# ericehanley/gke-ray-train

Measured on AMD Instinct MI355X. Metric: tokens/sec (whole node) Llama-2-7B fine-tune at 1/2/4/8 MI355X; samples/sec on Wikitext-2, higher is better.
Workload: dtype bf16; 1 GPU; model=llama2-7b, global_batch=8, seq_len=1024, parallelism=dp1, micro_batch=8, grad_accum=1, optimizer=fused AdamW fp32 states, activation_checkpointing=False, optimizer_overlap=True, forced_collectives=False, library_gemms=offline-tuned

## Files before the change

### gke_ray_train_amd/csrc/bindings/ops.cpp

```cpp
#include <climits>
#include <torch/extension.h>

#include <algorithm>
#include <cmath>
#include <c10/hip/HIPStream.h>
#include <c10/core/DeviceGuard.h>

#include "grt_kernels.h"
#include "grt_sdma.h"

namespace {

using at::Tensor;
using c10::optional;

hipStream_t cur_stream(const Tensor& t) {
  return c10::hip::getCurrentHIPStream(t.device().index()).stream();
}

grt::DType dtype_of(const Tensor& t) {
  if (t.scalar_type() == at::kBFloat16) return grt::DType::BF16;
  TORCH_CHECK(t.scalar_type() == at::kFloat, "gke_ray_train_amd kernels support bf16/fp32, got ", t.scalar_type());
  return grt::DType::F32;
}
// ... 21 lines not shown
  check_vec(t, d, name);
  const int64_t vec = t.scalar_type() == at::kBFloat16 ? 8 : 4;
  TORCH_CHECK(d / vec <= grt::norm_max_chunks(), name, ": last dim ", d, " is wider than the norm kernels' limit of ",
              grt::norm_max_chunks(), " 16-byte chunks (", grt::norm_max_chunks() * vec, " elements of ",
              t.scalar_type(), ")");
  return d;
}
void check_norm_like(const Tensor& t, const Tensor& rows_t, const char* name) {
  check_contig(t, name);
  TORCH_CHECK(t.sizes() == rows_t.sizes() && t.scalar_type() == rows_t.scalar_type() && t.device() == rows_t.device(),
              name, " must match the input's shape, dtype and device");
}
void check_norm_param(const Tensor& t, const Tensor& rows_t, int64_t d, const char* name) {
  check_contig(t, name);
  TORCH_CHECK(t.numel() == d && t.scalar_type() == rows_t.scalar_type() && t.device() == rows_t.device(), name,
              " must hold ", d, " elements in the input's dtype on its device");
}
void check_norm_stat(const Tensor& t, const Tensor& rows_t, int64_t rows, const char* name) {
  check_contig(t, name);
  TORCH_CHECK(t.numel() == rows && t.scalar_type() == at::kFloat && t.device() == rows_t.device(), name,
              " must hold one fp32 value per row (", rows, ") on the input's device");
}

std::vector<Tensor> rmsnorm_fwd(const Tensor& x, const optional<Tensor>& residual, const Tensor& w,
                                double eps, int64_t pad) {
  const int64_t d = check_norm_rows(x, "x"), rows = x.numel() / d;
  check_norm_param(w, x, d, "w");
  c10::OptionalDeviceGuard g(x.device());
  TORCH_CHECK(pad >= 0 && pad % 8 == 0 && (pad == 0 || x.dim() == 2), "rmsnorm_fwd: pad % 8 == 0 on [rows, d]");
  auto y = pad == 0 ? at::empty_like(x) : at::empty({rows, d + pad}, x.options()).narrow(1, 0, d);
  auto rstd = at::empty({rows}, x.options().dtype(at::kFloat));
  Tensor h;
  if (residual.has_value()) {
    check_norm_like(*residual, x, "residual");
    h = at::empty_like(x);
  }
  if (rows == 0) return {y, residual.has_value() ? h : x, rstd};
  grt::rmsnorm_fwd(dtype_of(x), x.data_ptr(), ptr_or_null(residual), w.data_ptr(), y.data_ptr(),
                   residual.has_value() ? h.data_ptr() : nullptr, rstd.data_ptr<float>(), rows, (int)d,
                   (float)eps, cur_stream(x), d + pad);
  return {y, residual.has_value() ? h : x, rstd};
}

std::vector<Tensor> rmsnorm_bwd(const Tensor& dy, const Tensor& h, const Tensor& w, const Tensor& rstd,
                                const optional<Tensor>& dres, const optional<Tensor>& dw_out, bool accumulate) {
  const int64_t d = check_norm_rows(h, "h"), rows = h.numel() / d;
  check_norm_like(dy, h, "dy");
  check_norm_param(w, h, d, "w");
  check_norm_stat(rstd, h, rows, "rstd");
  if (dres.has_value()) check_norm_like(*dres, h, "dres");
  if (dw_out.has_value()) check_norm_param(*dw_out, h, d, "dw_out");
  c10::OptionalDeviceGuard g(h.device());
  auto dx = at::empty_like(h);
  if (rows == 0) {
    if (!dw_out.has_value()) return {dx, at::zeros({d}, h.options().dtype(at::kFloat))};
    if (!accumulate) dw_out->zero_();
    return {dx, *dw_out};
  }
  Tensor dw = dw_out.has_value() ? *dw_out : at::empty({d}, h.options().dtype(at::kFloat));
  auto ws = at::empty({grt::norm_bwd_workspace_floats(rows, (int)d)}, h.options().dtype(at::kFloat));
  grt::rmsnorm_bwd(dtype_of(h), dy.data_ptr(), h.data_ptr(), w.data_ptr(), rstd.data_ptr<float>(),
                   ptr_or_null(dres), dx.data_ptr(), dw_out.has_value() ? nullptr : dw.data_ptr<float>(),
                   ws.data_ptr<float>(), rows, (int)d, cur_stream(h),
                   dw_out.has_value() ? dw.data_ptr() : nullptr, accumulate ? 1 : 0);
  return {dx, dw};
}

Tensor rmsnorm_bwd_dx(const Tensor& dy, const Tensor& h, const Tensor& w, const Tensor& rstd,
                      const optional<Tensor>& dres) {
  const int64_t d = check_norm_rows(h, "h"), rows = h.numel() / d;
  check_norm_like(dy, h, "dy");
  check_norm_param(w, h, d, "w");
  check_norm_stat(rstd, h, rows, "rstd");
  if (dres.has_value()) check_norm_like(*dres, h, "dres");
  c10::OptionalDeviceGuard g(h.device());
  auto dx = at::empty_like(h);
  if (rows == 0) return dx;
  grt::rmsnorm_bwd(dtype_of(h), dy.data_ptr(), h.data_ptr(), w.data_ptr(), rstd.data_ptr<float>(),
                   ptr_or_null(dres), dx.data_ptr(), nullptr, nullptr, rows, (int)d, cur_stream(h), nullptr, 0);
  return dx;
}

std::vector<Tensor> layernorm_fwd(const Tensor& x, const optional<Tensor>& residual, const Tensor& w,
                                  const optional<Tensor>& b, double eps) {
  const int64_t d = check_norm_rows(x, "x"), rows = x.numel() / d;
  check_norm_param(w, x, d, "w");
  if (b.has_value()) check_norm_param(*b, x, d, "b");
  c10::OptionalDeviceGuard g(x.device());
  auto y = at::empty_like(x);
  auto mean = at::empty({rows}, x.options().dtype(at::kFloat));
  auto rstd = at::empty({rows}, x.options().dtype(at::kFloat));
  Tensor h;
  if (residual.has_value()) {
    check_norm_like(*residual, x, "residual");
    h = at::empty_like(x);
  }
  if (rows == 0) return {y, residual.has_value() ? h : x, mean, rstd};
  grt::layernorm_fwd(dtype_of(x), x.data_ptr(), ptr_or_null(residual), w.data_ptr(), ptr_or_null(b),
                     y.data_ptr(), residual.has_value() ? h.data_ptr() : nullptr, mean.data_ptr<float>(),
                     rstd.data_ptr<float>(), rows, (int)d, (float)eps, cur_stream(x));
  return {y, residual.has_value() ? h : x, mean, rstd};
}

std::vector<Tensor> layernorm_bwd(const Tensor& dy, const Tensor& h, const Tensor& w, const Tensor& mean,
                                  const Tensor& rstd, const optional<Tensor>& dres) {
  const int64_t d = check_norm_rows(h, "h"), rows = h.numel() / d;
  check_norm_like(dy, h, "dy");
  check_norm_param(w, h, d, "w");
  check_norm_stat(mean, h, rows, "mean");
  check_norm_stat(rstd, h, rows, "rstd");
  if (dres.has_value()) check_norm_like(*dres, h, "dres");
  c10::OptionalDeviceGuard g(h.device());
  auto dx = at::empty_like(h);
  if (rows == 0) {
    auto z = at::zeros({d}, h.options().dtype(at::kFloat));
    return {dx, z, at::zeros_like(z)};
  }
  auto dw = at::empty({d}, h.options().dtype(at::kFloat));
  auto db = at::empty({d}, h.options().dtype(at::kFloat));
  auto ws = at::empty({grt::norm_bwd_workspace_floats(rows, (int)d)}, h.options().dtype(at::kFloat));
  grt::layernorm_bwd(dtype_of(h), dy.data_ptr(), h.data_ptr(), w.data_ptr(), mean.data_ptr<float>(),
                     rstd.data_ptr<float>(), ptr_or_null(dres), dx.data_ptr(), dw.data_ptr<float>(),
                     db.data_ptr<float>(), ws.data_ptr<float>(), rows, (int)d, cur_stream(h));
  return {dx, dw, db};
}

Tensor swiglu_fwd(const Tensor& gu, int64_t pad) {
  check_contig(gu, "gu");
  c10::OptionalDeviceGuard g(gu.device());
  const int64_t two_f = gu.size(-1), rows = gu.numel() / two_f, f = two_f / 2;
  check_vec(gu, f, "gu");
  TORCH_CHECK(pad >= 0 && pad % 8 == 0 && (pad == 0 || gu.dim() == 2), "swiglu_fwd: pad % 8 == 0 on [rows, 2f]");
  auto sizes = gu.sizes().vec();
  sizes.back() = f;
  auto out = pad == 0 ? at::empty(sizes, gu.options()) : at::empty({rows, f + pad}, gu.options()).narrow(1, 0, f);
  grt::swiglu_fwd(dtype_of(gu), gu.data_ptr(), out.data_ptr(), rows, (int)f, cur_stream(gu), f + pad);
  return out;
}
Tensor swiglu_bwd(const Tensor& gu, const Tensor& dout) {
  check_contig(gu, "gu");
  check_contig(dout, "dout");
  c10::OptionalDeviceGuard g(gu.device());
  const int64_t two_f = gu.size(-1), rows = gu.numel() / two_f, f = two_f / 2;
// ... 1630 lines not shown
    any = any || words[i] != 0;
  }
  TORCH_CHECK(any, "cu_masked_stream: mask selects no CU");
  c10::DeviceGuard g(c10::Device(c10::DeviceType::CUDA, (c10::DeviceIndex)device));
  hipStream_t s = nullptr;
  const hipError_t e = hipExtStreamCreateWithCUMask(&s, (uint32_t)words.size(), words.data());
  TORCH_CHECK(e == hipSuccess, "hipExtStreamCreateWithCUMask: ", hipGetErrorString(e));
  return reinterpret_cast<int64_t>(s);
}

std::vector<int64_t> stream_cu_mask(int64_t stream, int64_t words) {
  TORCH_CHECK(words > 0 && words <= 64, "stream_cu_mask: 1..64 words");
  std::vector<uint32_t> w((size_t)words, 0u);
  const hipError_t e = hipExtStreamGetCUMask(reinterpret_cast<hipStream_t>(stream), (uint32_t)words, w.data());
  TORCH_CHECK(e == hipSuccess, "hipExtStreamGetCUMask: ", hipGetErrorString(e));
  return std::vector<int64_t>(w.begin(), w.end());
}

}

PYBIND11_MODULE(TORCH_EXTENSION_NAME, m) {
  m.doc() = "gke_ray_train_amd HIP kernels for gfx950 (MI355X)";
  m.def("rmsnorm_fwd", &rmsnorm_fwd, py::arg("x"), py::arg("residual"), py::arg("w"), py::arg("eps"),
        py::arg("pad") = 0);
  m.def("rmsnorm_bwd", &rmsnorm_bwd, py::arg("dy"), py::arg("h"), py::arg("w"), py::arg("rstd"), py::arg("dres"),
        py::arg("dw_out") = py::none(), py::arg("accumulate") = false);
  m.def("layernorm_fwd", &layernorm_fwd);
  m.def("layernorm_bwd", &layernorm_bwd);
  m.def("swiglu_fwd", &swiglu_fwd, py::arg("gu"), py::arg("pad") = 0);
  m.def("swiglu_bwd", &swiglu_bwd);
  m.def("gelu_fwd", &gelu_fwd);
  m.def("gelu_bwd", &gelu_bwd);
  m.def("rope_fwd", &rope_fwd);
  m.def("rope_bwd", &rope_bwd);
  m.def("rope_append", &rope_append);
  m.def("rope_append_fp8", &rope_append_fp8, py::arg("qkv"), py::arg("cos"), py::arg("sin"), py::arg("pos"), py::arg("hq"),
        py::arg("hkv"), py::arg("D"), py::arg("S"), py::arg("kc"), py::arg("vc"), py::arg("k_scale"), py::arg("v_scale"),
        py::arg("tpr"), py::arg("k_out") = py::none());
  m.def("kv_fp8_dequant", &kv_fp8_dequant);
  m.def("scale_add_pe", &scale_add_pe);
  m.def("dropout_fwd", &dropout_fwd);
  m.def("dropout_bwd", &dropout_bwd);
  m.def("dropout_fwd_seeded", &dropout_fwd_seeded);
  m.def("lora_down", &lora_down, py::arg("x"), py::arg("a"), py::arg("p"), py::arg("seed"), py::arg("offset"),
        py::arg("want_xd"), py::arg("h_out") = py::none(), py::arg("hscale") = 1.0);
  m.def("lora_dx", &lora_dx, py::arg("g"), py::arg("at"), py::arg("dx"), py::arg("p"), py::arg("seed"),
        py::arg("offset"), py::arg("accumulate"), py::arg("dx_in") = py::none(), py::arg("gscale") = 1.0);
  m.def("lora_refresh", &lora_refresh, py::arg("bs"), py::arg("offs"), py::arg("w"), py::arg("wt"), py::arg("col0"),
        py::arg("wt_row0") = -1);
  m.def("lora_g", &lora_g, py::arg("a"), py::arg("bt"), py::arg("c"), py::arg("alpha"), py::arg("accumulate"));
  m.def("lora_g_group", &lora_g_group, py::arg("a"), py::arg("bt"), py::arg("c"), py::arg("alpha"),
// ... 32 lines not shown
        py::arg("rope_sin") = py::none(), py::arg("cu_seqlens") = py::none(), py::arg("max_seqlen") = 0,
        py::arg("dqkv_t") = py::none());
  m.def("rope_attn_fwd_d64", &rope_attn_fwd_d64, py::arg("qkv"), py::arg("cos"), py::arg("sin"), py::arg("o"),
        py::arg("B"), py::arg("S"), py::arg("hq"), py::arg("hkv"), py::arg("scale"), py::arg("causal"),
        py::arg("cu_seqlens") = py::none(), py::arg("max_seqlen") = 0,
        "bf16 head_dim 64: RoPE + flash attention straight from the fused QKV rows (packed with cu_seqlens) -> lse");
  m.def("rope_attn_bwd_d64", &rope_attn_bwd_d64, py::arg("do"), py::arg("qkv"), py::arg("cos"), py::arg("sin"),
        py::arg("o"), py::arg("lse"), py::arg("dqkv"), py::arg("B"), py::arg("S"), py::arg("hq"), py::arg("hkv"),
        py::arg("scale"), py::arg("causal"), py::arg("cu_seqlens") = py::none(), py::arg("max_seqlen") = 0,
        "backward of rope_attn_fwd_d64: un-rotated dQ / dK and dV into the columns of dqkv (every element written)");
  m.def("attn_set_schedule", &grt::attn_set_schedule,
        "bf16 attention causal-pair / XCD-grouped schedule, bit mask: 1 = forward, 2 = dQ, 4 = dK/dV");
  m.def("attn_get_schedule", &grt::attn_get_schedule);
  m.def("attn_set_dkdv_form", &grt::attn_set_dkdv_form, "dK / dV kernel: 1 = 4-wave, 2 = wave-pair (default)");
  m.def("attn_get_dkdv_form", &grt::attn_get_dkdv_form);
  m.def("attn_set_dma_fast", &grt::attn_set_dma_fast, "1 = hoisted LDS-DMA addressing (default), 0 = clamped per tile");
  m.def("ew_set_fast", &grt::ew_set_fast, "1 = single-pass RoPE (D = 128) / SwiGLU kernels (default), 0 = grid-stride kernels");
  m.def("attn_set_skip_dead", &grt::attn_set_skip_dead,
        "1 = forward / dK-dV waves skip the causal tiles they mask entirely (default), 0 = compute them");
  m.def("nf4_quantize", &nf4_quantize);
  m.def("nf4_dequantize", &nf4_dequantize);
  m.def("nf4_dequantize_t", &nf4_dequantize_t);
  m.def("nf4_dequantize_into", &nf4_dequantize_into);
  m.def("rmsnorm_bwd_dx", &rmsnorm_bwd_dx);
  m.def("swiglu_fwd_t", &swiglu_fwd_t);
  m.def("swiglu_bwd_t", &swiglu_bwd_t);
  m.def("transpose_into", &transpose_into);
  m.def("copy_sdma", &copy_sdma);
  m.def("sdma_d2h", &sdma_d2h, py::arg("dst"), py::arg("src"), py::arg("producer_stream") = 0,
        "pinned host <- device on an SDMA engine, ordered on the source's current stream; producer_stream "
        "(a raw stream handle): the stream whose work so far wrote src");
  m.def("sdma_stats", &sdma_stats, "copies / bytes / worker busy seconds / first error of the SDMA copier");
  m.def("sdma_clear_error", [](int64_t device) { grt::sdma_clear_error((int)device); });
  m.def("gemv", &gemv, py::arg("x"), py::arg("w"), py::arg("swiglu") = false);
  m.def("gemv_fused", &gemv_fused, py::arg("x"), py::arg("w"), py::arg("sumsq"), py::arg("slot"),
        py::arg("swiglu") = false, py::arg("g") = py::none(), py::arg("res") = py::none(), py::arg("eps") = 1e-5,
        py::arg("cos") = py::none(), py::arg("sin") = py::none(), py::arg("pos") = py::none(),
        py::arg("kc") = py::none(), py::arg("vc") = py::none(), py::arg("hq") = 0, py::arg("hkv") = 0);
  m.def("nf4_gemv", &nf4_gemv, py::arg("x"), py::arg("qweight"), py::arg("absmax"), py::arg("N"), py::arg("K"),
        py::arg("h") = py::none(), py::arg("lora_b") = py::none(), py::arg("lora_off") = py::none(),
        py::arg("scaling") = 1.0);
  m.def("sample_logits", &sample_logits, py::arg("logits"), py::arg("do_sample") = false, py::arg("temperature") = 1.0,
        py::arg("top_k") = 0, py::arg("top_p") = 1.0, py::arg("seed") = 0, py::arg("counter") = py::none(),
        py::arg("keep_mask") = py::none(), py::arg("finished") = py::none(), py::arg("finish_step") = py::none(),
        py::arg("step") = py::none(), py::arg("next_ids") = py::none(), py::arg("out") = py::none(),
        py::arg("eos_ids") = py::none(), py::arg("pad_id") = py::none(), py::arg("max_steps") = 1,
        py::arg("candidates") = false);
// ... 34 lines not shown
```

### gke_ray_train_amd/csrc/include/grt_kernels.h

```cpp
#pragma once
#include <hip/hip_runtime.h>
#include <stdint.h>

namespace grt {

enum class DType : int { F32 = 0, BF16 = 1 };

void rmsnorm_fwd(DType dt, const void* x, const void* residual, const void* w, void* y, void* h_out,
                 float* rstd, int64_t rows, int d, float eps, hipStream_t s,
                 int64_t ldy = 0);
void rmsnorm_bwd(DType dt, const void* dy, const void* h, const void* w, const float* rstd,
                 const void* dres, void* dx, float* dw_f32, float* ws, int64_t rows, int d,
                 hipStream_t s, void* dw_t = nullptr, int accumulate = 0);
int64_t norm_bwd_workspace_floats(int64_t rows, int d);
int norm_max_chunks();
void layernorm_fwd(DType dt, const void* x, const void* residual, const void* w, const void* b,
                   void* y, void* h_out, float* mean, float* rstd, int64_t rows, int d, float eps,
                   hipStream_t s);
void layernorm_bwd(DType dt, const void* dy, const void* h, const void* w, const float* mean,
                   const float* rstd, const void* dres, void* dx, float* dw_f32, float* db_f32,
                   float* ws, int64_t rows, int d, hipStream_t s);

void swiglu_fwd(DType dt, const void* gu, void* out, int64_t rows, int f, hipStream_t s, int64_t ldo = 0);
bool swiglu_fwd_t(const void* gu, void* out, void* outT, int64_t rows, int f, hipStream_t s, int64_t ldo = 0);
bool swiglu_bwd_t(const void* gu, const void* dout, void* dgu, void* dguT, int64_t rows, int f, hipStream_t s);
void swiglu_bwd(DType dt, const void* gu, const void* dout, void* dgu, int64_t rows, int f,
                hipStream_t s);
void gelu_fwd(DType dt, const void* x, void* y, int64_t n, hipStream_t s);
void gelu_bwd(DType dt, const void* x, const void* dy, void* dx, int64_t n, hipStream_t s);
void ew_set_fast(int on);
void rope_fwd(DType dt, const void* qkv, int64_t ld, void* q_out, void* k_out, const float* cos,
              const float* sin, const int32_t* pos, int64_t T, int S, int hq, int hkv, int D,
              hipStream_t s);
void rope_append(const void* qkv, int64_t ld, void* q_out, void* kc, void* vc, int64_t c_bs, int64_t c_ss,
                 int64_t c_hs, int64_t v_bs, int64_t v_ss, int64_t v_hs, const float* cos, const float* sin,
                 const int32_t* pos, int64_t T_, int tpr, int S, int L, int hq, int hkv, int D, hipStream_t s);
void rope_bwd(DType dt, const void* dq, const void* dk, void* dqkv, int64_t ld, const float* cos,
// ... 344 lines not shown
```

### gke_ray_train_amd/csrc/kernels/norm.hip

```cpp
#include <stdlib.h>

#include "grt_common.h"
#include "grt_kernels.h"

namespace grt {
namespace {

constexpr int kNT = 256;
constexpr int kRowsPerBlock = kNT / kWave;
constexpr int kBwdMaxBlocks = 512;

template <typename T, int MAXC, bool RMS, bool RES, bool FULL>
__global__ __launch_bounds__(kNT) void norm_fwd_kernel(const T* __restrict__ x,
                                                       const T* __restrict__ res,
                                                       const T* __restrict__ w,
                                                       const T* __restrict__ b, T* __restrict__ y,
                                                       T* __restrict__ h_out, float* __restrict__ mean_out,
                                                       float* __restrict__ rstd_out, int64_t rows,
                                                       int d, float eps, int64_t ldy) {
  constexpr int V = Vec16<T>::N;
  typedef typename Vec16<T>::type VT;
  const int lane = threadIdx.x & 63;
  const int64_t row = (int64_t)blockIdx.x * kRowsPerBlock + (threadIdx.x >> 6);
  if (row >= rows) return;
  const int nchunk = d / V;
  const T* xr = x + row * d;
  const T* rr = RES ? res + row * d : nullptr;
  VT xv[MAXC], rv[MAXC], wvv[MAXC];
#pragma unroll
  for (int c = 0; c < MAXC; ++c) {
    const int ch = FULL ? lane + c * kWave : min(lane + c * kWave, nchunk - 1);
    xv[c] = *reinterpret_cast<const VT*>(xr + ch * V);
    if (RES) rv[c] = *reinterpret_cast<const VT*>(rr + ch * V);
  }
#pragma unroll
  for (int c = 0; c < MAXC; ++c) {
    const int ch = FULL ? lane + c * kWave : min(lane + c * kWave, nchunk - 1);
    wvv[c] = *reinterpret_cast<const VT*>(w + ch * V);
  }
  float hv[MAXC][V];
  float s1 = 0.f;
#pragma unroll
  for (int c = 0; c < MAXC; ++c) {
    const bool ok = FULL || lane + c * kWave < nchunk;
#pragma unroll
    for (int i = 0; i < V; ++i) {
      float t = to_f(xv[c][i]);
      if (RES) t = to_f(from_f<T>(t + to_f(rv[c][i])));
      hv[c][i] = ok ? t : 0.f;
      s1 += RMS ? hv[c][i] * hv[c][i] : hv[c][i];
    }
    if (RES && ok) store16(h_out + row * d + (lane + c * kWave) * V, hv[c]);
  }
  s1 = wave_sum(s1);
  float mu = 0.f, rstd;
  if (RMS) {
    rstd = rsqrtf(s1 / d + eps);
  } else {
    mu = s1 / d;
    float s2 = 0.f;
#pragma unroll
    for (int c = 0; c < MAXC; ++c) {
      const bool ok = FULL || lane + c * kWave < nchunk;
#pragma unroll
      for (int i = 0; i < V; ++i) { const float t = hv[c][i] - mu; s2 += ok ? t * t : 0.f; }
    }
    s2 = wave_sum(s2);
    rstd = rsqrtf(s2 / d + eps);
  }
#pragma unroll
  for (int c = 0; c < MAXC; ++c) {
    const int ch = lane + c * kWave;
    if (FULL || ch < nchunk) {
      float o[V];
      if (!RMS && b != nullptr) {
        float bv[V];
        load16(b + ch * V, bv);
#pragma unroll
        for (int i = 0; i < V; ++i) o[i] = (hv[c][i] - mu) * rstd * to_f(wvv[c][i]) + bv[i];
      } else {
#pragma unroll
        for (int i = 0; i < V; ++i) o[i] = (hv[c][i] - mu) * rstd * to_f(wvv[c][i]);
      }
      store16(y + row * ldy + ch * V, o);
    }
  }
  if (lane == 0) {
    rstd_out[row] = rstd;
    if (!RMS) mean_out[row] = mu;
  }
}

template <typename T, int MAXC, bool RMS, bool RES>
__global__ __launch_bounds__(kNT) void norm_bwd_kernel(const T* __restrict__ dy,
                                                       const T* __restrict__ h,
                                                       const T* __restrict__ w,
                                                       const float* __restrict__ mean,
                                                       const float* __restrict__ rstd,
                                                       const T* __restrict__ dres, T* __restrict__ dx,
                                                       float* __restrict__ ws, int64_t rows, int d) {
  constexpr int V = Vec16<T>::N;
  typedef typename Vec16<T>::type VT;
  __shared__ float red[2 * kRowsPerBlock];
  const int tid = threadIdx.x, lane = tid & 63, wid = tid >> 6;
  const int nchunk = d / V;
  float dwp[MAXC][V], dbp[MAXC][V], wv[MAXC][V];
  int chs[MAXC];
#pragma unroll
  for (int c = 0; c < MAXC; ++c) {
    chs[c] = min(tid + c * kNT, nchunk - 1);
#pragma unroll
    for (int i = 0; i < V; ++i) { dwp[c][i] = 0.f; dbp[c][i] = 0.f; }
    load16(w + chs[c] * V, wv[c]);
  }
  VT hn[MAXC], dn[MAXC], rn[MAXC];
  auto load_row = [&](int64_t rr) {
    rr = rr < rows ? rr : rows - 1;
#pragma unroll
    for (int c = 0; c < MAXC; ++c) {
      hn[c] = *reinterpret_cast<const VT*>(h + rr * d + chs[c] * V);
      dn[c] = *reinterpret_cast<const VT*>(dy + rr * d + chs[c] * V);
      if (RES) rn[c] = *reinterpret_cast<const VT*>(dres + rr * d + chs[c] * V);
    }
  };
  load_row(blockIdx.x);
  for (int64_t row = blockIdx.x; row < rows; row += gridDim.x) {
    VT hc[MAXC], dc[MAXC], rc[MAXC];
#pragma unroll
    for (int c = 0; c < MAXC; ++c) { hc[c] = hn[c]; dc[c] = dn[c]; if (RES) rc[c] = rn[c]; }
    load_row(row + gridDim.x);
    const float r = rstd[row];
    const float mu = RMS ? 0.f : mean[row];
    float xh[MAXC][V], g[MAXC][V];
    float sg = 0.f, sgx = 0.f;
#pragma unroll
    for (int c = 0; c < MAXC; ++c) {
      const bool ok = tid + c * kNT < nchunk;
#pragma unroll
      for (int i = 0; i < V; ++i) {
        const float dv = ok ? to_f(dc[c][i]) : 0.f;
        xh[c][i] = (to_f(hc[c][i]) - mu) * r;
        g[c][i] = dv * wv[c][i];
        sg += g[c][i];
        sgx += g[c][i] * xh[c][i];
        dwp[c][i] += dv * xh[c][i];
        if (!RMS) dbp[c][i] += dv;
      }
    }
    sgx = wave_sum(sgx);
    if (!RMS) sg = wave_sum(sg);
    if (lane == 0) { red[wid] = sgx; red[kRowsPerBlock + wid] = sg; }
    __syncthreads();
    float tsgx = 0.f, tsg = 0.f;
#pragma unroll
    for (int i = 0; i < kRowsPerBlock; ++i) { tsgx += red[i]; tsg += red[kRowsPerBlock + i]; }
    __syncthreads();
    tsgx /= d;
    tsg = RMS ? 0.f : tsg / d;
#pragma unroll
    for (int c = 0; c < MAXC; ++c) {
      const int ch = tid + c * kNT;
      if (ch < nchunk) {
        float o[V];
#pragma unroll
        for (int i = 0; i < V; ++i) o[i] = (RES ? to_f(rc[c][i]) : 0.f) + r * (g[c][i] - tsg - xh[c][i] * tsgx);
        store16(dx + row * d + ch * V, o);
      }
    }
  }
  if (ws == nullptr) return;
  float* wsb = ws + (int64_t)blockIdx.x * 2 * d;
#pragma unroll
  for (int c = 0; c < MAXC; ++c) {
    const int ch = tid + c * kNT;
    if (ch < nchunk) {
#pragma unroll
      for (int i = 0; i < V; ++i) {
        wsb[ch * V + i] = dwp[c][i];
        wsb[d + ch * V + i] = dbp[c][i];
      }
    }
  }
}

constexpr int kColsumCols = 16;
constexpr int kColsumGroups = kNT / kColsumCols;
template <typename GO, bool ACC>
__global__ __launch_bounds__(kNT) void colsum_kernel(const float* __restrict__ ws, int nb, int d, int ncols,
                                                     GO* __restrict__ dw, GO* __restrict__ db) {
  __shared__ float red[kColsumGroups][kColsumCols];
  const int c = threadIdx.x % kColsumCols, rg = threadIdx.x / kColsumCols;
  const int j = blockIdx.x * kColsumCols + c;
  float a0 = 0.f, a1 = 0.f, a2 = 0.f, a3 = 0.f;
  if (j < ncols) {
    const int64_t ld = 2 * (int64_t)d;
    constexpr int G = kColsumGroups;
    int b = rg;
    for (; b + 3 * G < nb; b += 4 * G) {
      a0 += ws[(int64_t)b * ld + j];
      a1 += ws[(int64_t)(b + G) * ld + j];
      a2 += ws[(int64_t)(b + 2 * G) * ld + j];
      a3 += ws[(int64_t)(b + 3 * G) * ld + j];
    }
    for (; b < nb; b += G) a0 += ws[(int64_t)b * ld + j];
  }
  red[rg][c] = (a0 + a1) + (a2 + a3);
  __syncthreads();
  if (rg == 0 && j < ncols) {
    float s = 0.f;
#pragma unroll
    for (int g = 0; g < kColsumGroups; ++g) s += red[g][c];
    GO* out = j < d ? dw : db;
    const int jj = j < d ? j : j - d;
    if (out) out[jj] = from_f<GO>(ACC ? to_f(out[jj]) + s : s);
  }
}

constexpr int kNormMaxFwdPerLane = 32;
constexpr int kNormMaxBwdPerThr = 8;
constexpr int kNormMaxChunks = kNormMaxFwdPerLane * kWave;
static_assert(kNormMaxChunks == kNormMaxBwdPerThr * kNT, "forward and backward ladders cover the same width");

template <typename T, bool RMS>
void launch_fwd(const void* x, const void* res, const void* w, const void* b, void* y, void* h_out,
                float* mean, float* rstd, int64_t rows, int d, float eps, hipStream_t s, int64_t ldy = 0) {
  if (ldy <= 0) ldy = d;
  constexpr int V = Vec16<T>::N;
  const int per_lane = (d / V + kWave - 1) / kWave;
  const dim3 grid((unsigned)((rows + kRowsPerBlock - 1) / kRowsPerBlock));
#define GRT_NF4(MC, RES, FULL)                                                                  \
  hipLaunchKernelGGL((norm_fwd_kernel<T, MC, RMS, RES, FULL>), grid, dim3(kNT), 0, s, (const T*)x, \
                     (const T*)res, (const T*)w, (const T*)b, (T*)y, (T*)h_out, mean, rstd, rows,     \
                     d, eps, ldy)
#define GRT_NF(MC)                                                     \
  do {                                                                 \
    const bool full = (d / V) == (MC) * kWave;                         \
    if (res != nullptr) { if (full) GRT_NF4(MC, true, true); else GRT_NF4(MC, true, false); }   \
    else { if (full) GRT_NF4(MC, false, true); else GRT_NF4(MC, false, false); }              \
  } while (0)
  if (per_lane <= 1) GRT_NF(1);
  else if (per_lane <= 2) GRT_NF(2);
  else if (per_lane <= 4) GRT_NF(4);
  else if (per_lane <= 8) GRT_NF(8);
  else if (per_lane <= 16) GRT_NF(16);
  else GRT_NF(kNormMaxFwdPerLane);
#undef GRT_NF
#undef GRT_NF4
}

int bwd_max_blocks() {
  static const int v = [] {
    const char* e = getenv("GRT_NORM_BWD_BLOCKS");
    const int n = e ? atoi(e) : kBwdMaxBlocks;
    return n > 0 ? n : kBwdMaxBlocks;
  }();
  return v;
}

int bwd_blocks(int64_t rows) {
  const int mb = bwd_max_blocks();
  return (int)(rows < mb ? (rows > 0 ? rows : 1) : mb);
}

template <typename T, bool RMS>
void launch_bwd(const void* dy, const void* h, const void* w, const float* mean, const float* rstd,
                const void* dres, void* dx, float* dw, float* db, float* ws, int64_t rows, int d,
                hipStream_t s, void* dw_t = nullptr, int accumulate = 0) {
  constexpr int V = Vec16<T>::N;
  const int per_thr = (d / V + kNT - 1) / kNT;
  const int nb = bwd_blocks(rows);
  const size_t lds = 0;
#define GRT_NB2(MC, RES)                                                                            \
  hipLaunchKernelGGL((norm_bwd_kernel<T, MC, RMS, RES>), dim3(nb), dim3(kNT), lds, s, (const T*)dy, \
                     (const T*)h, (const T*)w, mean, rstd, (const T*)dres, (T*)dx, ws, rows, d)
#define GRT_NB(MC)                                      \
  do {                                                  \
    if (dres != nullptr) GRT_NB2(MC, true);             \
    else GRT_NB2(MC, false);                            \
  } while (0)
  if (per_thr <= 1) GRT_NB(1);
  else if (per_thr <= 2) GRT_NB(2);
  else if (per_thr <= 4) GRT_NB(4);
  else GRT_NB(kNormMaxBwdPerThr);
#undef GRT_NB
#undef GRT_NB2
  if (ws == nullptr) return;
  const int ncols = RMS ? d : 2 * d;
  const dim3 cg((ncols + kColsumCols - 1) / kColsumCols);
  if (dw_t != nullptr && RMS) {
    if (accumulate)
      hipLaunchKernelGGL((colsum_kernel<T, true>), cg, dim3(kNT), 0, s, ws, nb, d, ncols, (T*)dw_t, (T*)nullptr);
    else
      hipLaunchKernelGGL((colsum_kernel<T, false>), cg, dim3(kNT), 0, s, ws, nb, d, ncols, (T*)dw_t, (T*)nullptr);
  } else {
    hipLaunchKernelGGL((colsum_kernel<float, false>), cg, dim3(kNT), 0, s, ws, nb, d, ncols, dw, db);
  }
}

}

int norm_max_chunks() { return kNormMaxChunks; }

int64_t norm_bwd_workspace_floats(int64_t rows, int d) { return (int64_t)bwd_blocks(rows) * 2 * d; }

void rmsnorm_fwd(DType dt, const void* x, const void* residual, const void* w, void* y, void* h_out,
                 float* rstd, int64_t rows, int d, float eps, hipStream_t s, int64_t ldy) {
  if (dt == DType::BF16)
    launch_fwd<bf16, true>(x, residual, w, nullptr, y, h_out, nullptr, rstd, rows, d, eps, s, ldy);
  else
    launch_fwd<float, true>(x, residual, w, nullptr, y, h_out, nullptr, rstd, rows, d, eps, s, ldy);
}

void rmsnorm_bwd(DType dt, const void* dy, const void* h, const void* w, const float* rstd,
                 const void* dres, void* dx, float* dw_f32, float* ws, int64_t rows, int d,
                 hipStream_t s, void* dw_t, int accumulate) {
  if (dt == DType::BF16)
    launch_bwd<bf16, true>(dy, h, w, nullptr, rstd, dres, dx, dw_f32, nullptr, ws, rows, d, s, dw_t, accumulate);
  else
    launch_bwd<float, true>(dy, h, w, nullptr, rstd, dres, dx, dw_f32, nullptr, ws, rows, d, s, dw_t, accumulate);
}

void layernorm_fwd(DType dt, const void* x, const void* residual, const void* w, const void* b,
                   void* y, void* h_out, float* mean, float* rstd, int64_t rows, int d, float eps,
                   hipStream_t s) {
  if (dt == DType::BF16)
    launch_fwd<bf16, false>(x, residual, w, b, y, h_out, mean, rstd, rows, d, eps, s);
// ... 15 lines not shown
```

Before: 28060 tokens/s.

## Make norm kernels persistent with row prefetch, multi-row bwd, vectorized colsum

The forward norm kernel now runs on a capped persistent grid, prefetching the next row's inputs while the current row reduces. It also keeps the residual sum in bf16 registers instead of fp32. The backward kernel handles two rows per iteration for small widths, compiles out the dw path when no workspace is given, and stores only the dw half of the workspace for RMSNorm. The column-sum kernel switches to 1024 threads with float4 loads and shuffle reductions. Optional output buffers are added to the bindings so callers can reuse allocations; this adds register pressure and more complex code paths in the norm kernels, which are a small share of step time.

```diff
diff --git a/gke_ray_train_amd/csrc/bindings/ops.cpp b/gke_ray_train_amd/csrc/bindings/ops.cpp
--- a/gke_ray_train_amd/csrc/bindings/ops.cpp
+++ b/gke_ray_train_amd/csrc/bindings/ops.cpp
@@ -67,18 +67,27 @@
               " must hold one fp32 value per row (", rows, ") on the input's device");
 }
 
+Tensor norm_out(const optional<Tensor>& out, const Tensor& rows_t, const char* name) {
+  if (!out.has_value()) return at::empty_like(rows_t);
+  check_norm_like(*out, rows_t, name);
+  TORCH_CHECK(reinterpret_cast<uintptr_t>(out->data_ptr()) % 16 == 0, name, " must be 16-byte aligned");
+  return *out;
+}
+
 std::vector<Tensor> rmsnorm_fwd(const Tensor& x, const optional<Tensor>& residual, const Tensor& w,
-                                double eps, int64_t pad) {
+                                double eps, int64_t pad, const optional<Tensor>& y_out,
+                                const optional<Tensor>& h_out) {
   const int64_t d = check_norm_rows(x, "x"), rows = x.numel() / d;
   check_norm_param(w, x, d, "w");
   c10::OptionalDeviceGuard g(x.device());
   TORCH_CHECK(pad >= 0 && pad % 8 == 0 && (pad == 0 || x.dim() == 2), "rmsnorm_fwd: pad % 8 == 0 on [rows, d]");
-  auto y = pad == 0 ? at::empty_like(x) : at::empty({rows, d + pad}, x.options()).narrow(1, 0, d);
+  TORCH_CHECK(pad == 0 || !y_out.has_value(), "rmsnorm_fwd: y_out only with pad == 0");
+  auto y = pad == 0 ? norm_out(y_out, x, "y_out") : at::empty({rows, d + pad}, x.options()).narrow(1, 0, d);
   auto rstd = at::empty({rows}, x.options().dtype(at::kFloat));
   Tensor h;
   if (residual.has_value()) {
     check_norm_like(*residual, x, "residual");
-    h = at::empty_like(x);
+    h = norm_out(h_out, x, "h_out");
   }
   if (rows == 0) return {y, residual.has_value() ? h : x, rstd};
   grt::rmsnorm_fwd(dtype_of(x), x.data_ptr(), ptr_or_null(residual), w.data_ptr(), y.data_ptr(),
@@ -88,7 +97,8 @@
 }
 
 std::vector<Tensor> rmsnorm_bwd(const Tensor& dy, const Tensor& h, const Tensor& w, const Tensor& rstd,
-                                const optional<Tensor>& dres, const optional<Tensor>& dw_out, bool accumulate) {
+                                const optional<Tensor>& dres, const optional<Tensor>& dw_out, bool accumulate,
+                                const optional<Tensor>& dx_out) {
   const int64_t d = check_norm_rows(h, "h"), rows = h.numel() / d;
   check_norm_like(dy, h, "dy");
   check_norm_param(w, h, d, "w");
@@ -96,14 +106,14 @@
   if (dres.has_value()) check_norm_like(*dres, h, "dres");
   if (dw_out.has_value()) check_norm_param(*dw_out, h, d, "dw_out");
   c10::OptionalDeviceGuard g(h.device());
-  auto dx = at::empty_like(h);
+  auto dx = norm_out(dx_out, h, "dx_out");
   if (rows == 0) {
     if (!dw_out.has_value()) return {dx, at::zeros({d}, h.options().dtype(at::kFloat))};
     if (!accumulate) dw_out->zero_();
     return {dx, *dw_out};
   }
   Tensor dw = dw_out.has_value() ? *dw_out : at::empty({d}, h.options().dtype(at::kFloat));
-  auto ws = at::empty({grt::norm_bwd_workspace_floats(rows, (int)d)}, h.options().dtype(at::kFloat));
+  auto ws = at::empty({grt::norm_bwd_workspace_floats(rows, (int)d, true)}, h.options().dtype(at::kFloat));
   grt::rmsnorm_bwd(dtype_of(h), dy.data_ptr(), h.data_ptr(), w.data_ptr(), rstd.data_ptr<float>(),
                    ptr_or_null(dres), dx.data_ptr(), dw_out.has_value() ? nullptr : dw.data_ptr<float>(),
                    ws.data_ptr<float>(), rows, (int)d, cur_stream(h),
@@ -112,33 +122,37 @@
 }
 
 Tensor rmsnorm_bwd_dx(const Tensor& dy, const Tensor& h, const Tensor& w, const Tensor& rstd,
-                      const optional<Tensor>& dres) {
+                      const optional<Tensor>& dres, const optional<Tensor>& dx_out) {
   const int64_t d = check_norm_rows(h, "h"), rows = h.numel() / d;
   check_norm_like(dy, h, "dy");
   check_norm_param(w, h, d, "w");
   check_norm_stat(rstd, h, rows, "rstd");
   if (dres.has_value()) check_norm_like(*dres, h, "dres");
   c10::OptionalDeviceGuard g(h.device());
-  auto dx = at::empty_like(h);
+  auto dx = norm_out(dx_out, h, "dx_out");
   if (rows == 0) return dx;
   grt::rmsnorm_bwd(dtype_of(h), dy.data_ptr(), h.data_ptr(), w.data_ptr(), rstd.data_ptr<float>(),
                    ptr_or_null(dres), dx.data_ptr(), nullptr, nullptr, rows, (int)d, cur_stream(h), nullptr, 0);
   return dx;
 }
 
+int64_t norm_fwd_max_waves() { return grt::norm_fwd_max_waves(); }
+int64_t norm_bwd_blocks(int64_t rows) { return grt::norm_bwd_blocks(rows); }
+
 std::vector<Tensor> layernorm_fwd(const Tensor& x, const optional<Tensor>& residual, const Tensor& w,
-                                  const optional<Tensor>& b, double eps) {
+                                  const optional<Tensor>& b, double eps, const optional<Tensor>& y_out,
+                                  const optional<Tensor>& h_out) {
   const int64_t d = check_norm_rows(x, "x"), rows = x.numel() / d;
   check_norm_param(w, x, d, "w");
   if (b.has_value()) check_norm_param(*b, x, d, "b");
   c10::OptionalDeviceGuard g(x.device());
-  auto y = at::empty_like(x);
+  auto y = norm_out(y_out, x, "y_out");
   auto mean = at::empty({rows}, x.options().dtype(at::kFloat));
   auto rstd = at::empty({rows}, x.options().dtype(at::kFloat));
   Tensor h;
   if (residual.has_value()) {
     check_norm_like(*residual, x, "residual");
-    h = at::empty_like(x);
+    h = norm_out(h_out, x, "h_out");
   }
   if (rows == 0) return {y, residual.has_value() ? h : x, mean, rstd};
   grt::layernorm_fwd(dtype_of(x), x.data_ptr(), ptr_or_null(residual), w.data_ptr(), ptr_or_null(b),
@@ -148,7 +162,7 @@
 }
 
 std::vector<Tensor> layernorm_bwd(const Tensor& dy, const Tensor& h, const Tensor& w, const Tensor& mean,
-                                  const Tensor& rstd, const optional<Tensor>& dres) {
+                                  const Tensor& rstd, const optional<Tensor>& dres, const optional<Tensor>& dx_out) {
   const int64_t d = check_norm_rows(h, "h"), rows = h.numel() / d;
   check_norm_like(dy, h, "dy");
   check_norm_param(w, h, d, "w");
@@ -156,14 +170,14 @@
   check_norm_stat(rstd, h, rows, "rstd");
   if (dres.has_value()) check_norm_like(*dres, h, "dres");
   c10::OptionalDeviceGuard g(h.device());
-  auto dx = at::empty_like(h);
+  auto dx = norm_out(dx_out, h, "dx_out");
   if (rows == 0) {
     auto z = at::zeros({d}, h.options().dtype(at::kFloat));
     return {dx, z, at::zeros_like(z)};
   }
   auto dw = at::empty({d}, h.options().dtype(at::kFloat));
   auto db = at::empty({d}, h.options().dtype(at::kFloat));
-  auto ws = at::empty({grt::norm_bwd_workspace_floats(rows, (int)d)}, h.options().dtype(at::kFloat));
+  auto ws = at::empty({grt::norm_bwd_workspace_floats(rows, (int)d, false)}, h.options().dtype(at::kFloat));
   grt::layernorm_bwd(dtype_of(h), dy.data_ptr(), h.data_ptr(), w.data_ptr(), mean.data_ptr<float>(),
                      rstd.data_ptr<float>(), ptr_or_null(dres), dx.data_ptr(), dw.data_ptr<float>(),
                      db.data_ptr<float>(), ws.data_ptr<float>(), rows, (int)d, cur_stream(h));
@@ -1840,11 +1854,15 @@
 PYBIND11_MODULE(TORCH_EXTENSION_NAME, m) {
   m.doc() = "gke_ray_train_amd HIP kernels for gfx950 (MI355X)";
   m.def("rmsnorm_fwd", &rmsnorm_fwd, py::arg("x"), py::arg("residual"), py::arg("w"), py::arg("eps"),
-        py::arg("pad") = 0);
+        py::arg("pad") = 0, py::arg("y_out") = py::none(), py::arg("h_out") = py::none());
   m.def("rmsnorm_bwd", &rmsnorm_bwd, py::arg("dy"), py::arg("h"), py::arg("w"), py::arg("rstd"), py::arg("dres"),
-        py::arg("dw_out") = py::none(), py::arg("accumulate") = false);
-  m.def("layernorm_fwd", &layernorm_fwd);
-  m.def("layernorm_bwd", &layernorm_bwd);
+        py::arg("dw_out") = py::none(), py::arg("accumulate") = false, py::arg("dx_out") = py::none());
+  m.def("layernorm_fwd", &layernorm_fwd, py::arg("x"), py::arg("residual"), py::arg("w"), py::arg("b"), py::arg("eps"),
+        py::arg("y_out") = py::none(), py::arg("h_out") = py::none());
+  m.def("norm_fwd_max_waves", &norm_fwd_max_waves);
+  m.def("norm_bwd_blocks", &norm_bwd_blocks);
+  m.def("layernorm_bwd", &layernorm_bwd, py::arg("dy"), py::arg("h"), py::arg("w"), py::arg("mean"), py::arg("rstd"),
+        py::arg("dres"), py::arg("dx_out") = py::none());
   m.def("swiglu_fwd", &swiglu_fwd, py::arg("gu"), py::arg("pad") = 0);
   m.def("swiglu_bwd", &swiglu_bwd);
   m.def("gelu_fwd", &gelu_fwd);
@@ -1923,7 +1941,8 @@
   m.def("nf4_dequantize", &nf4_dequantize);
   m.def("nf4_dequantize_t", &nf4_dequantize_t);
   m.def("nf4_dequantize_into", &nf4_dequantize_into);
-  m.def("rmsnorm_bwd_dx", &rmsnorm_bwd_dx);
+  m.def("rmsnorm_bwd_dx", &rmsnorm_bwd_dx, py::arg("dy"), py::arg("h"), py::arg("w"), py::arg("rstd"), py::arg("dres"),
+        py::arg("dx_out") = py::none());
   m.def("swiglu_fwd_t", &swiglu_fwd_t);
   m.def("swiglu_bwd_t", &swiglu_bwd_t);
   m.def("transpose_into", &transpose_into);
diff --git a/gke_ray_train_amd/csrc/include/grt_kernels.h b/gke_ray_train_amd/csrc/include/grt_kernels.h
--- a/gke_ray_train_amd/csrc/include/grt_kernels.h
+++ b/gke_ray_train_amd/csrc/include/grt_kernels.h
@@ -12,7 +12,9 @@
 void rmsnorm_bwd(DType dt, const void* dy, const void* h, const void* w, const float* rstd,
                  const void* dres, void* dx, float* dw_f32, float* ws, int64_t rows, int d,
                  hipStream_t s, void* dw_t = nullptr, int accumulate = 0);
-int64_t norm_bwd_workspace_floats(int64_t rows, int d);
+int64_t norm_bwd_workspace_floats(int64_t rows, int d, bool rms);
+int norm_bwd_blocks(int64_t rows);
+int norm_fwd_max_waves();
 int norm_max_chunks();
 void layernorm_fwd(DType dt, const void* x, const void* residual, const void* w, const void* b,
                    void* y, void* h_out, float* mean, float* rstd, int64_t rows, int d, float eps,
diff --git a/gke_ray_train_amd/csrc/kernels/norm.hip b/gke_ray_train_amd/csrc/kernels/norm.hip
--- a/gke_ray_train_amd/csrc/kernels/norm.hip
+++ b/gke_ray_train_amd/csrc/kernels/norm.hip
@@ -9,6 +9,14 @@
 constexpr int kNT = 256;
 constexpr int kRowsPerBlock = kNT / kWave;
 constexpr int kBwdMaxBlocks = 512;
+constexpr int kFwdMaxBlocks = 512;
+
+template <typename VT>
+__device__ __forceinline__ void use16(VT& v) {
+  u32x4 t = __builtin_bit_cast(u32x4, v);
+  asm volatile("" : "+v"(t));
+  v = __builtin_bit_cast(VT, t);
+}
 
 template <typename T, int MAXC, bool RMS, bool RES, bool FULL>
 __global__ __launch_bounds__(kNT) void norm_fwd_kernel(const T* __restrict__ x,
@@ -20,78 +28,99 @@
                                                        int d, float eps, int64_t ldy) {
   constexpr int V = Vec16<T>::N;
   typedef typename Vec16<T>::type VT;
+  constexpr bool PF = MAXC <= 8;
   const int lane = threadIdx.x & 63;
-  const int64_t row = (int64_t)blockIdx.x * kRowsPerBlock + (threadIdx.x >> 6);
+  const int64_t nwave = (int64_t)gridDim.x * kRowsPerBlock;
+  int64_t row = (int64_t)blockIdx.x * kRowsPerBlock + (threadIdx.x >> 6);
   if (row >= rows) return;
   const int nchunk = d / V;
-  const T* xr = x + row * d;
-  const T* rr = RES ? res + row * d : nullptr;
-  VT xv[MAXC], rv[MAXC], wvv[MAXC];
+  const bool bias = !RMS && b != nullptr;
+  int chs[MAXC];
+  VT xn[MAXC], rn[MAXC], wvv[MAXC], bvv[MAXC];
+#pragma unroll
+  for (int c = 0; c < MAXC; ++c) chs[c] = FULL ? lane + c * kWave : min(lane + c * kWave, nchunk - 1);
+  auto load_row = [&](int64_t r) {
+    r = r < rows ? r : rows - 1;
+#pragma unroll
+    for (int c = 0; c < MAXC; ++c) {
+      xn[c] = *reinterpret_cast<const VT*>(x + r * d + chs[c] * V);
+      if (RES) rn[c] = *reinterpret_cast<const VT*>(res + r * d + chs[c] * V);
+    }
+  };
 #pragma unroll
   for (int c = 0; c < MAXC; ++c) {
-    const int ch = FULL ? lane + c * kWave : min(lane + c * kWave, nchunk - 1);
-    xv[c] = *reinterpret_cast<const VT*>(xr + ch * V);
-    if (RES) rv[c] = *reinterpret_cast<const VT*>(rr + ch * V);
-  }
-#pragma unroll
-  for (int c = 0; c < MAXC; ++c) {
-    const int ch = FULL ? lane + c * kWave : min(lane + c * kWave, nchunk - 1);
-    wvv[c] = *reinterpret_cast<const VT*>(w + ch * V);
-  }
-  float hv[MAXC][V];
-  float s1 = 0.f;
-#pragma unroll
-  for (int c = 0; c < MAXC; ++c) {
-    const bool ok = FULL || lane + c * kWave < nchunk;
-#pragma unroll
-    for (int i = 0; i < V; ++i) {
-      float t = to_f(xv[c][i]);
-      if (RES) t = to_f(from_f<T>(t + to_f(rv[c][i])));
-      hv[c][i] = ok ? t : 0.f;
-      s1 += RMS ? hv[c][i] * hv[c][i] : hv[c][i];
-    }
-    if (RES && ok) store16(h_out + row * d + (lane + c * kWave) * V, hv[c]);
-  }
-  s1 = wave_sum(s1);
-  float mu = 0.f, rstd;
-  if (RMS) {
-    rstd = rsqrtf(s1 / d + eps);
-  } else {
-    mu = s1 / d;
-    float s2 = 0.f;
+    wvv[c] = *reinterpret_cast<const VT*>(w + chs[c] * V);
+    if (!RMS) bvv[c] = *reinterpret_cast<const VT*>((bias ? b : w) + chs[c] * V);
+  }
+  if (PF) {
+    load_row(row);
+#pragma unroll
+    for (int c = 0; c < MAXC; ++c) {
+      use16(xn[c]);
+      if (RES) use16(rn[c]);
+    }
+  }
+  for (; row < rows; row += nwave) {
+    if (!PF) load_row(row);
+    VT hb[MAXC];
+    float s1 = 0.f;
 #pragma unroll
     for (int c = 0; c < MAXC; ++c) {
       const bool ok = FULL || lane + c * kWave < nchunk;
 #pragma unroll
-      for (int i = 0; i < V; ++i) { const float t = hv[c][i] - mu; s2 += ok ? t * t : 0.f; }
-    }
-    s2 = wave_sum(s2);
-    rstd = rsqrtf(s2 / d + eps);
-  }
-#pragma unroll
-  for (int c = 0; c < MAXC; ++c) {
-    const int ch = lane + c * kWave;
-    if (FULL || ch < nchunk) {
-      float o[V];
-      if (!RMS && b != nullptr) {
-        float bv[V];
-        load16(b + ch * V, bv);
-#pragma unroll
-        for (int i = 0; i < V; ++i) o[i] = (hv[c][i] - mu) * rstd * to_f(wvv[c][i]) + bv[i];
-      } else {
-#pragma unroll
-        for (int i = 0; i < V; ++i) o[i] = (hv[c][i] - mu) * rstd * to_f(wvv[c][i]);
-      }
-      store16(y + row * ldy + ch * V, o);
-    }
-  }
-  if (lane == 0) {
-    rstd_out[row] = rstd;
-    if (!RMS) mean_out[row] = mu;
-  }
-}
-
-template <typename T, int MAXC, bool RMS, bool RES>
+      for (int i = 0; i < V; ++i) {
+        float t = to_f(xn[c][i]);
+        if (RES) t = to_f(from_f<T>(t + to_f(rn[c][i])));
+        t = ok ? t : 0.f;
+        hb[c][i] = from_f<T>(t);
+        s1 += RMS ? t * t : t;
+      }
+      if (RES && ok) *reinterpret_cast<VT*>(h_out + row * d + (lane + c * kWave) * V) = hb[c];
+    }
+    if (PF) {
+      __builtin_amdgcn_sched_barrier(0);
+      load_row(row + nwave);
+      __builtin_amdgcn_sched_barrier(0);
+    }
+    s1 = wave_sum(s1);
+    float mu = 0.f, rstd;
+    if (RMS) {
+      rstd = rsqrtf(s1 / d + eps);
+    } else {
+      mu = s1 / d;
+      float s2 = 0.f;
+#pragma unroll
+      for (int c = 0; c < MAXC; ++c) {
+        const bool ok = FULL || lane + c * kWave < nchunk;
+#pragma unroll
+        for (int i = 0; i < V; ++i) { const float t = to_f(hb[c][i]) - mu; s2 += ok ? t * t : 0.f; }
+      }
+      s2 = wave_sum(s2);
+      rstd = rsqrtf(s2 / d + eps);
+    }
+#pragma unroll
+    for (int c = 0; c < MAXC; ++c) {
+      const int ch = lane + c * kWave;
+      if (FULL || ch < nchunk) {
+        float o[V];
+        if (bias) {
+#pragma unroll
+          for (int i = 0; i < V; ++i) o[i] = (to_f(hb[c][i]) - mu) * rstd * to_f(wvv[c][i]) + to_f(bvv[c][i]);
+        } else {
+#pragma unroll
+          for (int i = 0; i < V; ++i) o[i] = (to_f(hb[c][i]) - mu) * rstd * to_f(wvv[c][i]);
+        }
+        store16(y + row * ldy + ch * V, o);
+      }
+    }
+    if (lane == 0) {
+      rstd_out[row] = rstd;
+      if (!RMS) mean_out[row] = mu;
+    }
+  }
+}
+
+template <typename T, int MAXC, bool RMS, bool RES, bool DW>
 __global__ __launch_bounds__(kNT) void norm_bwd_kernel(const T* __restrict__ dy,
                                                        const T* __restrict__ h,
                                                        const T* __restrict__ w,
@@ -100,10 +129,12 @@
                                                        const T* __restrict__ dres, T* __restrict__ dx,
                                                        float* __restrict__ ws, int64_t rows, int d) {
   constexpr int V = Vec16<T>::N;
+  constexpr int NR = MAXC <= 2 ? 2 : 1;
   typedef typename Vec16<T>::type VT;
-  __shared__ float red[2 * kRowsPerBlock];
+  __shared__ float red[2 * NR * kRowsPerBlock];
   const int tid = threadIdx.x, lane = tid & 63, wid = tid >> 6;
   const int nchunk = d / V;
+  const int64_t G = gridDim.x;
   float dwp[MAXC][V], dbp[MAXC][V], wv[MAXC][V];
   int chs[MAXC];
 #pragma unroll
@@ -113,63 +144,100 @@
     for (int i = 0; i < V; ++i) { dwp[c][i] = 0.f; dbp[c][i] = 0.f; }
     load16(w + chs[c] * V, wv[c]);
   }
-  VT hn[MAXC], dn[MAXC], rn[MAXC];
-  auto load_row = [&](int64_t rr) {
-    rr = rr < rows ? rr : rows - 1;
-#pragma unroll
-    for (int c = 0; c < MAXC; ++c) {
-      hn[c] = *reinterpret_cast<const VT*>(h + rr * d + chs[c] * V);
-      dn[c] = *reinterpret_cast<const VT*>(dy + rr * d + chs[c] * V);
-      if (RES) rn[c] = *reinterpret_cast<const VT*>(dres + rr * d + chs[c] * V);
+  VT hn[NR][MAXC], dn[NR][MAXC], rn[NR][MAXC];
+  auto load_rows = [&](int64_t r0) {
+#pragma unroll
+    for (int k = 0; k < NR; ++k) {
+      int64_t rr = r0 + k * G;
+      rr = rr < rows ? rr : rows - 1;
+#pragma unroll
+      for (int c = 0; c < MAXC; ++c) {
+        hn[k][c] = *reinterpret_cast<const VT*>(h + rr * d + chs[c] * V);
+        dn[k][c] = *reinterpret_cast<const VT*>(dy + rr * d + chs[c] * V);
+        if (RES) rn[k][c] = *reinterpret_cast<const VT*>(dres + rr * d + chs[c] * V);
+      }
     }
   };
-  load_row(blockIdx.x);
-  for (int64_t row = blockIdx.x; row < rows; row += gridDim.x) {
-    VT hc[MAXC], dc[MAXC], rc[MAXC];
-#pragma unroll
-    for (int c = 0; c < MAXC; ++c) { hc[c] = hn[c]; dc[c] = dn[c]; if (RES) rc[c] = rn[c]; }
-    load_row(row + gridDim.x);
-    const float r = rstd[row];
-    const float mu = RMS ? 0.f : mean[row];
-    float xh[MAXC][V], g[MAXC][V];
-    float sg = 0.f, sgx = 0.f;
-#pragma unroll
-    for (int c = 0; c < MAXC; ++c) {
-      const bool ok = tid + c * kNT < nchunk;
-#pragma unroll
-      for (int i = 0; i < V; ++i) {
-        const float dv = ok ? to_f(dc[c][i]) : 0.f;
-        xh[c][i] = (to_f(hc[c][i]) - mu) * r;
-        g[c][i] = dv * wv[c][i];
-        sg += g[c][i];
-        sgx += g[c][i] * xh[c][i];
-        dwp[c][i] += dv * xh[c][i];
-        if (!RMS) dbp[c][i] += dv;
-      }
-    }
-    sgx = wave_sum(sgx);
-    if (!RMS) sg = wave_sum(sg);
-    if (lane == 0) { red[wid] = sgx; red[kRowsPerBlock + wid] = sg; }
+  load_rows(blockIdx.x);
+  for (int64_t row = blockIdx.x; row < rows; row += NR * G) {
+    VT hc[NR][MAXC], dc[NR][MAXC], rc[NR][MAXC];
+#pragma unroll
+    for (int k = 0; k < NR; ++k) {
+#pragma unroll
+      for (int c = 0; c < MAXC; ++c) { hc[k][c] = hn[k][c]; dc[k][c] = dn[k][c]; if (RES) rc[k][c] = rn[k][c]; }
+    }
+    load_rows(row + NR * G);
+    float r[NR], mu[NR], sg[NR], sgx[NR];
+    float xh[NR][MAXC][V], g[NR][MAXC][V];
+#pragma unroll
+    for (int k = 0; k < NR; ++k) {
+      const bool live = row + k * G < rows;
+      const int64_t rk = live ? row + k * G : row;
+      r[k] = rstd[rk];
+      mu[k] = RMS ? 0.f : mean[rk];
+      sg[k] = 0.f;
+      sgx[k] = 0.f;
+#pragma unroll
+      for (int c = 0; c < MAXC; ++c) {
+        const bool ok = tid + c * kNT < nchunk;
+#pragma unroll
+        for (int i = 0; i < V; ++i) {
+          const float dv = ok ? to_f(dc[k][c][i]) : 0.f;
+          xh[k][c][i] = (to_f(hc[k][c][i]) - mu[k]) * r[k];
+          g[k][c][i] = dv * wv[c][i];
+          sg[k] += g[k][c][i];
+          sgx[k] += g[k][c][i] * xh[k][c][i];
+          if (DW) {
+            const float nw = dwp[c][i] + dv * xh[k][c][i];
+            dwp[c][i] = live ? nw : dwp[c][i];
+            if (!RMS) dbp[c][i] = live ? dbp[c][i] + dv : dbp[c][i];
+          }
+        }
+      }
+      sgx[k] = wave_sum(sgx[k]);
+      if (!RMS) sg[k] = wave_sum(sg[k]);
+    }
+    if (lane == 0) {
+#pragma unroll
+      for (int k = 0; k < NR; ++k) {
+        red[(2 * k) * kRowsPerBlock + wid] = sgx[k];
+        red[(2 * k + 1) * kRowsPerBlock + wid] = sg[k];
+      }
+    }
     __syncthreads();
-    float tsgx = 0.f, tsg = 0.f;
-#pragma unroll
-    for (int i = 0; i < kRowsPerBlock; ++i) { tsgx += red[i]; tsg += red[kRowsPerBlock + i]; }
+    float tsgx[NR], tsg[NR];
+#pragma unroll
+    for (int k = 0; k < NR; ++k) {
+      tsgx[k] = 0.f;
+      tsg[k] = 0.f;
+#pragma unroll
+      for (int i = 0; i < kRowsPerBlock; ++i) {
+        tsgx[k] += red[(2 * k) * kRowsPerBlock + i];
+        tsg[k] += red[(2 * k + 1) * kRowsPerBlock + i];
+      }
+    }
     __syncthreads();
-    tsgx /= d;
-    tsg = RMS ? 0.f : tsg / d;
-#pragma unroll
-    for (int c = 0; c < MAXC; ++c) {
-      const int ch = tid + c * kNT;
-      if (ch < nchunk) {
-        float o[V];
-#pragma unroll
-        for (int i = 0; i < V; ++i) o[i] = (RES ? to_f(rc[c][i]) : 0.f) + r * (g[c][i] - tsg - xh[c][i] * tsgx);
-        store16(dx + row * d + ch * V, o);
-      }
-    }
-  }
-  if (ws == nullptr) return;
-  float* wsb = ws + (int64_t)blockIdx.x * 2 * d;
+#pragma unroll
+    for (int k = 0; k < NR; ++k) {
+      if (row + k * G >= rows) break;
+      tsgx[k] /= d;
+      tsg[k] = RMS ? 0.f : tsg[k] / d;
+#pragma unroll
+      for (int c = 0; c < MAXC; ++c) {
+        const int ch = tid + c * kNT;
+        if (ch < nchunk) {
+          float o[V];
+#pragma unroll
+          for (int i = 0; i < V; ++i)
+            o[i] = (RES ? to_f(rc[k][c][i]) : 0.f) + r[k] * (g[k][c][i] - tsg[k] - xh[k][c][i] * tsgx[k]);
+          store16(dx + (row + k * G) * d + ch * V, o);
+        }
+      }
+    }
+  }
+  if (!DW) return;
+  const int ld = RMS ? d : 2 * d;
+  float* wsb = ws + (int64_t)blockIdx.x * ld;
 #pragma unroll
   for (int c = 0; c < MAXC; ++c) {
     const int ch = tid + c * kNT;
@@ -177,39 +245,43 @@
 #pragma unroll
       for (int i = 0; i < V; ++i) {
         wsb[ch * V + i] = dwp[c][i];
-        wsb[d + ch * V + i] = dbp[c][i];
-      }
-    }
-  }
-}
-
-constexpr int kColsumCols = 16;
-constexpr int kColsumGroups = kNT / kColsumCols;
+        if (!RMS) wsb[d + ch * V + i] = dbp[c][i];
+      }
+    }
+  }
+}
+
+constexpr int kColsumNT = 1024;
+constexpr int kColsumCols = 64;
+constexpr int kColsumWaves = kColsumNT / kWave;
+constexpr int kColsumGroups = kColsumNT / (kColsumCols / 4);
 template <typename GO, bool ACC>
-__global__ __launch_bounds__(kNT) void colsum_kernel(const float* __restrict__ ws, int nb, int d, int ncols,
-                                                     GO* __restrict__ dw, GO* __restrict__ db) {
-  __shared__ float red[kColsumGroups][kColsumCols];
-  const int c = threadIdx.x % kColsumCols, rg = threadIdx.x / kColsumCols;
-  const int j = blockIdx.x * kColsumCols + c;
-  float a0 = 0.f, a1 = 0.f, a2 = 0.f, a3 = 0.f;
-  if (j < ncols) {
-    const int64_t ld = 2 * (int64_t)d;
-    constexpr int G = kColsumGroups;
-    int b = rg;
-    for (; b + 3 * G < nb; b += 4 * G) {
-      a0 += ws[(int64_t)b * ld + j];
-      a1 += ws[(int64_t)(b + G) * ld + j];
-      a2 += ws[(int64_t)(b + 2 * G) * ld + j];
-      a3 += ws[(int64_t)(b + 3 * G) * ld + j];
-    }
-    for (; b < nb; b += G) a0 += ws[(int64_t)b * ld + j];
-  }
-  red[rg][c] = (a0 + a1) + (a2 + a3);
+__global__ __launch_bounds__(kColsumNT) void colsum_kernel(const float* __restrict__ ws, int nb, int d, int ncols,
+                                                           int ld, GO* __restrict__ dw, GO* __restrict__ db) {
+  __shared__ float red[kColsumWaves][kColsumCols];
+  const int lane = threadIdx.x & 63, wid = threadIdx.x >> 6;
+  const int cq = lane & 15, rg = wid * 4 + (lane >> 4);
+  const int j4 = blockIdx.x * kColsumCols + cq * 4;
+  f32x4 a = {0.f, 0.f, 0.f, 0.f};
+  if (j4 < ncols) {
+#pragma unroll 8
+    for (int b = rg; b < nb; b += kColsumGroups) a += *reinterpret_cast<const f32x4*>(ws + (int64_t)b * ld + j4);
+  }
+#pragma unroll
+  for (int i = 0; i < 4; ++i) {
+    a[i] += __shfl_xor(a[i], 16, kWave);
+    a[i] += __shfl_xor(a[i], 32, kWave);
+  }
+  if (lane < 16) {
+#pragma unroll
+    for (int i = 0; i < 4; ++i) red[wid][cq * 4 + i] = a[i];
+  }
   __syncthreads();
-  if (rg == 0 && j < ncols) {
+  const int j = blockIdx.x * kColsumCols + threadIdx.x;
+  if (threadIdx.x < kColsumCols && j < ncols) {
     float s = 0.f;
 #pragma unroll
-    for (int g = 0; g < kColsumGroups; ++g) s += red[g][c];
+    for (int g = 0; g < kColsumWaves; ++g) s += red[g][threadIdx.x];
     GO* out = j < d ? dw : db;
     const int jj = j < d ? j : j - d;
     if (out) out[jj] = from_f<GO>(ACC ? to_f(out[jj]) + s : s);
@@ -227,7 +299,8 @@
   if (ldy <= 0) ldy = d;
   constexpr int V = Vec16<T>::N;
   const int per_lane = (d / V + kWave - 1) / kWave;
-  const dim3 grid((unsigned)((rows + kRowsPerBlock - 1) / kRowsPerBlock));
+  const int64_t want = (rows + kRowsPerBlock - 1) / kRowsPerBlock;
+  const dim3 grid((unsigned)(want < kFwdMaxBlocks ? want : kFwdMaxBlocks));
 #define GRT_NF4(MC, RES, FULL)                                                                  \
   hipLaunchKernelGGL((norm_fwd_kernel<T, MC, RMS, RES, FULL>), grid, dim3(kNT), 0, s, (const T*)x, \
                      (const T*)res, (const T*)w, (const T*)b, (T*)y, (T*)h_out, mean, rstd, rows,     \
@@ -270,9 +343,14 @@
   const int per_thr = (d / V + kNT - 1) / kNT;
   const int nb = bwd_blocks(rows);
   const size_t lds = 0;
-#define GRT_NB2(MC, RES)                                                                            \
-  hipLaunchKernelGGL((norm_bwd_kernel<T, MC, RMS, RES>), dim3(nb), dim3(kNT), lds, s, (const T*)dy, \
+#define GRT_NB3(MC, RES, DW)                                                                            \
+  hipLaunchKernelGGL((norm_bwd_kernel<T, MC, RMS, RES, DW>), dim3(nb), dim3(kNT), lds, s, (const T*)dy, \
                      (const T*)h, (const T*)w, mean, rstd, (const T*)dres, (T*)dx, ws, rows, d)
+#define GRT_NB2(MC, RES)                                \
+  do {                                                  \
+    if (ws != nullptr) GRT_NB3(MC, RES, true);          \
+    else GRT_NB3(MC, RES, false);                       \
+  } while (0)
 #define GRT_NB(MC)                                      \
   do {                                                  \
     if (dres != nullptr) GRT_NB2(MC, true);             \
@@ -284,16 +362,17 @@
   else GRT_NB(kNormMaxBwdPerThr);
 #undef GRT_NB
 #undef GRT_NB2
+#undef GRT_NB3
   if (ws == nullptr) return;
-  const int ncols = RMS ? d : 2 * d;
+  const int ncols = RMS ? d : 2 * d, ld = ncols;
   const dim3 cg((ncols + kColsumCols - 1) / kColsumCols);
   if (dw_t != nullptr && RMS) {
     if (accumulate)
-      hipLaunchKernelGGL((colsum_kernel<T, true>), cg, dim3(kNT), 0, s, ws, nb, d, ncols, (T*)dw_t, (T*)nullptr);
+      hipLaunchKernelGGL((colsum_kernel<T, true>), cg, dim3(kColsumNT), 0, s, ws, nb, d, ncols, ld, (T*)dw_t, (T*)nullptr);
     else
-      hipLaunchKernelGGL((colsum_kernel<T, false>), cg, dim3(kNT), 0, s, ws, nb, d, ncols, (T*)dw_t, (T*)nullptr);
+      hipLaunchKernelGGL((colsum_kernel<T, false>), cg, dim3(kColsumNT), 0, s, ws, nb, d, ncols, ld, (T*)dw_t, (T*)nullptr);
   } else {
-    hipLaunchKernelGGL((colsum_kernel<float, false>), cg, dim3(kNT), 0, s, ws, nb, d, ncols, dw, db);
+    hipLaunchKernelGGL((colsum_kernel<float, false>), cg, dim3(kColsumNT), 0, s, ws, nb, d, ncols, ld, dw, db);
   }
 }
 
@@ -301,7 +380,13 @@
 
 int norm_max_chunks() { return kNormMaxChunks; }
 
-int64_t norm_bwd_workspace_floats(int64_t rows, int d) { return (int64_t)bwd_blocks(rows) * 2 * d; }
+int norm_fwd_max_waves() { return kFwdMaxBlocks * kRowsPerBlock; }
+
+int norm_bwd_blocks(int64_t rows) { return bwd_blocks(rows); }
+
+int64_t norm_bwd_workspace_floats(int64_t rows, int d, bool rms) {
+  return (int64_t)bwd_blocks(rows) * (rms ? d : 2 * d);
+}
 
 void rmsnorm_fwd(DType dt, const void* x, const void* residual, const void* w, void* y, void* h_out,
                  float* rstd, int64_t rows, int d, float eps, hipStream_t s, int64_t ldy) {
```

Measured after the change: 28080 tokens/s, median of 4. No clear change (+0.1%).
